# google/sentencepiece

Hardware: AMD Instinct MI355X
Metric: sentences/sec EncodeBatch, 32k unigram, MI355X (higher is better)
Workload: dtype u8 text -> i32 ids; f64 add / f32 store in the Viterbi relax

## Files before the change

sentencepiece_amd/csrc/api.cc:

```cpp
#include <hip/hip_runtime.h>

#include <cstdio>
#include <cstdlib>
#include <fcntl.h>
#include <sys/mman.h>
#include <sys/stat.h>
#include <sys/syscall.h>
#include <unistd.h>

#include <algorithm>
#include <cmath>
#include <condition_variable>
#include <cstring>
#include <fstream>
#include <functional>
#include <map>
#include <memory>
#include <mutex>
#include <thread>
#include <new>
#include <sstream>
#include <atomic>
#include <chrono>
#include <string>
// ... 281 lines not shown
  uint32_t dyn_list_cap = kDynListCapDefault;
  uint64_t nbest_budget = 32ull << 30;
  uint32_t nbest_hyps_min = 4096;
  uint32_t tile_min_lanes = 1;
  int32_t dx_npre = 0, dx_nsuf = 0, dx_pre[kMaxExtra] = {0}, dx_suf[kMaxExtra] = {0};
  bool dx_reverse = false;
  bool dx_unk = false;
  uint32_t compact_staged = 2048;
  bool no_direct = false;
  int fork_cus = 0;
  int fork_waves = 4;
  bool early_tail = false;
  bool no_overlap = false;
  bool no_ids16 = false;
  bool no_scan = false;
  bool no_word_dyn = false;
  bool memo_unsafe = false;
  bool force_word_dp = false;
  bool no_split = false;
  uint32_t split_min_raw = 576;
  bool split_own_launch = false;
  uint32_t split_tiles = 1;
  uint32_t split_per_byte = 4;
  uint32_t compact_big = kCompactBigIds;
  bool uw_exact = false;
  int uw_pipe = 1;
  bool no_uni_wave = false;
  uint32_t uni_wave_max = 0;
  int word_wgs = 1;
  uint64_t table_bytes = 0;
  uint64_t dn_table_bytes = 0;
  double load_ms = 0.0;
  int word_form = 3;
  int wordwave_waves = 14;
  int word_waves = 12;
  int tile_waves_override = 0;
  uint32_t lane_general_min_lanes = 0;
  uint32_t sub_buckets = kSubBuckets;
  int host_threads = 24;
  uint64_t host_chunk = 0;
  int reserve_cus = 0;
  uint32_t ring_override = 0;
  uint64_t stream_scratch_limit = 16ull << 30;
  bool wide_tcap = false;
  uint32_t main_max_raw = kStreamMainMaxRaw;
  LengthClass classes[kNumClasses];
};

namespace {

int Fail(spmx_handle *, int code, const std::string &msg) {
  t_error = msg;
  return code;
}
int FailHip(spmx_handle *h, hipError_t e, const char *what) {
  return Fail(h, kInternal, std::string(what) + ": " + hipGetErrorString(e));
}

#define HIP_OR_RETURN(h, expr)                                   \
  do {                                                           \
    hipError_t e_ = (expr);                                      \
    if (e_ != hipSuccess) return FailHip((h), e_, #expr);        \
  } while (0)

struct Lease {
  spmx_handle *h;
  std::unique_ptr<Workspace> ws;
// ... 385 lines not shown
  const bool fast_ok = StreamFastEligible(h->dev.flags) && !h->no_fast;
  const bool uds = (h->dev.flags & kNfHasUserDefined) != 0;
  uint32_t rcaps[kMaxClasses] = {0};
  for (int c = 0; c < ncls; ++c) rcaps[c] = cls[c].rcap;
  rcaps[ncls - 1] = cls[ncls - 1].rcap;
  const uint64_t max_raw = (0x7FFFFF00ull - 16) / h->dev.expand_max;
  auto record = [&](int slot, int which) -> hipError_t {
    return prof ? hipEventRecord(ws->ev[slot][which], stream) : hipSuccess;
  };
  auto scan_compact = [&]() -> int {
    ScanArgs sa{ws->d_counts.p, n32, ws->d_tile_sums.p, d_id_offsets};
    const uint32_t tiles = (n32 + kScanTile - 1) / kScanTile;
    HIP_OR_RETURN(h, LaunchScan(sa, static_cast<int>(tiles < static_cast<uint32_t>(wide) ? tiles : wide), stream));
    const uint32_t big = (n < 65536 || text_bytes > 160ull * n) ? h->compact_big : 0u;
    if (big) HIP_OR_RETURN(h, hipMemsetAsync(&ws->d_ctrl->big_count[0], 0, sizeof(uint32_t), stream));
    CompactArgs pa{ws->d_arena.p, ws->d_tmp_off.p, ws->d_counts.p, d_id_offsets, d_ids, d_ids ? ids_capacity : 0, n32, &ws->d_ctrl->status, h->compact_staged,
                   big, ws->d_big_list.p, &ws->d_ctrl->big_count[0]};
    const uint64_t cblocks = (n + 63) / 64;
    const uint64_t cgrid = cblocks < static_cast<uint64_t>(h->n_cu) * 32 ? cblocks : static_cast<uint64_t>(h->n_cu) * 32;
    HIP_OR_RETURN(h, LaunchCompact(pa, static_cast<int>(cgrid), stream));
    if (big) HIP_OR_RETURN(h, LaunchCompactBig(pa, h->n_cu * 4, stream));
    HIP_OR_RETURN(h, hipMemcpyAsync(ws->h_ctrl, ws->d_ctrl, offsetof(Ctrl, total_ids), hipMemcpyDeviceToHost, stream));
    HIP_OR_RETURN(h, hipMemcpyAsync(&ws->h_ctrl->total_ids, d_id_offsets + n, sizeof(uint64_t), hipMemcpyDeviceToHost, stream));
    HIP_OR_RETURN(h, hipStreamSynchronize(stream));
    return kOk;
  };
  uint64_t arena_cap_limit = 0;
  if (h->arena_first && arena_need > h->arena_first) { arena_need = h->arena_first; arena_cap_limit = h->arena_first; }
  const uint64_t arena_reserve = (h->arena_first || ws->reserve_text_bytes <= text_bytes) ? 0 :
      expand * ws->reserve_text_bytes + (10 + static_cast<uint64_t>(h->dev.n_prefix + h->dev.n_suffix)) * (ws->reserve_n > n ? ws->reserve_n : n) + 4096 +
      (direct ? (ws->reserve_text_bytes + (1 + static_cast<uint64_t>(h->dev.n_prefix + h->dev.n_suffix)) * (ws->reserve_n > n ? ws->reserve_n : n)) / (ids16 ? 2 : 1) + 8 : 0);
  for (int attempt = 0; attempt < 4; ++attempt) {
    uint64_t long_launches = 0;
    HIP_OR_RETURN(h, ws->d_arena.Reserve(arena_need > arena_reserve ? arena_need : arena_reserve));
    if (spans) HIP_OR_RETURN(h, ws->d_arena_tb.Reserve(ws->d_arena.cap));
    if (prof) HIP_OR_RETURN(h, hipEventRecord(ws->ev[kNumSlots][0], stream));
    HIP_OR_RETURN(h, hipMemsetAsync(ws->d_ctrl, 0, sizeof(Ctrl), stream));
    HIP_OR_RETURN(h, hipMemsetAsync(d_status, 0, n, stream));
    for (bool &u : ws->slot_used) u = false;
    uint32_t known[kMaxClasses] = {0};
    uint32_t gen_known[kMaxClasses] = {0};
    uint32_t align_known[kMaxClasses] = {0};
    uint64_t gen_total = 0;
    if (!direct) {
      if (int rc = RunClassify(h, ws, d_offsets, n32, stream, scanned ? d_text : nullptr, text_bytes, scanned ? gen_lists : nullptr); rc != kOk) return rc;
      HIP_OR_RETURN(h, hipMemcpyAsync(ws->h_ctrl->list_counts, ws->d_ctrl->list_counts,
                                      sizeof(ws->h_ctrl->list_counts) + sizeof(ws->h_ctrl->gen_counts),
                                      hipMemcpyDeviceToHost, stream));
      HIP_OR_RETURN(h, hipStreamSynchronize(stream));
      for (int c = 0; c < ncls; ++c) { known[c] = ws->h_ctrl->list_counts[c]; gen_known[c] = ws->h_ctrl->gen_counts[c]; gen_total += gen_known[c]; }
    } else {
      known[0] = n32;
    }
    EncodeArgs a{};
    a.dev = h->dev; a.text = d_text; a.offs = d_offsets;
    a.arena = ws->d_arena.p; a.arena_head = &ws->d_ctrl->arena_head;
    a.arena_cap = attempt == 0 && arena_cap_limit && arena_cap_limit < ws->d_arena.cap ? arena_cap_limit : ws->d_arena.cap;
    a.tmp_off = ws->d_tmp_off.p; a.counts = ws->d_counts.p; a.sent_status = d_status; a.status = &ws->d_ctrl->status;
    a.arena_tb = spans ? ws->d_arena_tb.p : nullptr;
    a.long_list = long_list; a.side = &ws->d_ctrl->side;
    a.lists = class_lists; a.over_list = over_list;
    a.n = n32;
    a.fast_ok = fast_ok ? 1u : 0u;
    a.no_lane_general = h->no_lane_general ? 1u : 0u;
    a.no_char_norm = h->char_norm_mode;
    int stream_waves_cap = 0;
// ... 227 lines not shown
        }
        int rc = kOk;
        for (int c = 0; c < ncls && rc == kOk; ++c)
          if (doc_known[c]) rc = long_launch(class_lists + static_cast<size_t>(c) * n, &ws->d_ctrl->list_counts[c], doc_known[c], true);
        if (rc == kOk) rc = general_pass(gen_lists, ws->d_ctrl->gen_counts, gen_known, false);
        if (forked) {
          if (rc != kOk) { (void)hipStreamSynchronize(ws->stream2); return rc; }
          if (hipError_t e = hipEventRecord(ws->ev_join, stream); e != hipSuccess) { (void)hipStreamSynchronize(ws->stream2); return FailHip(h, e, "hipEventRecord(join)"); }
          stream = main_stream;
          stream_waves_cap = 0;
          stream_cus_cap = 0;
        } else if (rc != kOk) {
          return rc;
        }
        a.lists = class_lists;
        d_list_counts = ws->d_ctrl->list_counts;
      }
    }
    auto fail_forked = [&](int rc) -> int {
      if (forked) (void)hipStreamSynchronize(ws->stream2);
      return rc;
    };
#define FORKED_OR_RETURN(expr) do { if (int rc_ = (expr); rc_ != kOk) return fail_forked(rc_); } while (0)
#define FORKED_HIP_OR_RETURN(expr) do { hipError_t e_ = (expr); if (e_ != hipSuccess) return fail_forked(FailHip(h, e_, #expr)); } while (0)
    if (word_ok) {
      const bool dyn = !h->no_word_dyn;
      word_pass = [&](int mode, int slot, int qi, uint32_t *out_lists, uint32_t *d_out_counts, uint32_t *out2_lists,
                           uint32_t *d_out2_counts) -> int {
        const bool dp = mode == 3;
        EncodeArgs wa = a;
        const bool wform = !dp && ((mode == 2 ? h->word_form & 2 : h->word_form & 1) != 0);
        int waves = dp ? 8 : wform ? h->wordwave_waves : h->word_waves;
        if (wform && mode == 2 && waves > static_cast<int>(kWwAgainMaxWaves)) waves = static_cast<int>(kWwAgainMaxWaves);
        while (wform && waves > 1 && WordWaveLdsBytes(static_cast<uint32_t>(waves)) > 160u * 1024u) --waves;
        uint64_t total = 0;
        for (int c = 0; c < ncls; ++c) total += known[c];
        if (total == 0) return kOk;
        uint64_t grid = static_cast<uint64_t>(h->n_cu - h->reserve_cus) * static_cast<uint64_t>(dp ? 1 : h->word_wgs);
        if (grid * waves * 64 > total) grid = (total + waves * 64 - 1) / (waves * 64);
        if (grid < 1) grid = 1;
        const uint64_t n_waves = grid * waves;
        wa.n_classes = static_cast<uint32_t>(ncls);
        uint32_t tile_base = 0;
        wa.direct = direct ? 1u : 0u;
        if (direct && mode != 2) wa.lists = nullptr;
        for (int c = ncls - 1; c >= 0; --c) {
          StreamClass &sc = wa.cls[c];
          sc = StreamClass{};
          sc.rcap = rcaps[c];
          if (direct) {
            sc.lane_shift = 6;
            sc.general = cls[c].rcap > kMaxStagedRaw ? 1u : 0u;
            if (c == 0) {
              sc.count = static_cast<uint32_t>(total);
              sc.tw = 64;
              sc.main_tiles = static_cast<uint32_t>((total + 63) / 64);
              sc.tile_base = 0;
              tile_base = sc.main_tiles;
            }
            continue;
          }
          if (known[c] == 0) continue;
          uint64_t tw = (static_cast<uint64_t>(known[c]) + n_waves - 1) / n_waves;
          if (tw > 64) tw = 64;
          if (tw < 1) tw = 1;
          sc.lane_shift = 6;
          sc.general = ((uni_class[c] && cls[c].rcap > kMaxStagedRaw) || cls[c].rcap > h->main_max_raw) ? 1u : 0u;
          sc.count = known[c];
          sc.tw = static_cast<uint32_t>(tw);
          sc.main_tiles = static_cast<uint32_t>((static_cast<uint64_t>(known[c]) + tw - 1) / tw);
          sc.tile_base = tile_base;
          tile_base += sc.main_tiles;
        }
        wa.total_main = tile_base;
        wa.q = &ws->d_ctrl->q[qi];
        wa.stats = &ws->d_ctrl->stats[kStatsPerClass * slot];
        wa.left_lists = out_lists;
        wa.left_counts = d_out_counts;
        wa.left2_lists = out2_lists;
        wa.left2_counts = d_out2_counts;
        wa.dyn_tag = ws->d_dyn_tag.p;
        wa.dyn_ent = ws->d_dyn_ent.p;
        wa.dyn_list = ws->d_dyn_list.p;
        wa.dyn_count = &ws->d_ctrl->dyn_count;
        wa.dyn_mask = h->dyn_slots - 1u;
        wa.dyn_cap = h->dyn_list_cap;
        wa.resume = ws->d_resume.p;
        wa.ids16 = ids16 ? 1u : 0u;
        wa.arena_first = (direct && mode != 2) ? direct_region : 0u;
        snprintf(ws->slot_name[slot], sizeof(ws->slot_name[slot]), "%s",
                 wform ? (wa.ids16 ? (mode == 2 ? "EncodeWordWaveAgainKernel<true>" : mode == 1 ? "EncodeWordWaveCollectKernel<true>" : "EncodeWordWaveKernel<true>")
                                   : (mode == 2 ? "EncodeWordWaveAgainKernel<false>" : mode == 1 ? "EncodeWordWaveCollectKernel<false>" : "EncodeWordWaveKernel<false>"))
                       : mode == 3 ? "EncodeWordDpKernel" : mode == 2 ? "EncodeWordAgainKernel" : mode == 1 ? "EncodeWordCollectKernel" : "EncodeWordKernel");
        HIP_OR_RETURN(h, record(slot, 0));
        if (wform) HIP_OR_RETURN(h, LaunchEncodeWordWave(mode, wa, static_cast<int>(grid), waves, WordWaveLdsBytes(waves), stream));
        else HIP_OR_RETURN(h, LaunchEncodeWord(mode, wa, static_cast<int>(grid), waves, WordLdsBytes(waves, dp), stream));
        HIP_OR_RETURN(h, record(slot, 1));
        ws->slot_used[slot] = true;
        return kOk;
      };
      auto read_counts = [&]() -> int {
        HIP_OR_RETURN(h, hipMemcpyAsync(ws->h_ctrl->left_counts, ws->d_ctrl->left_counts, sizeof(ws->h_ctrl->left_counts) + sizeof(uint32_t),
                                        hipMemcpyDeviceToHost, stream));
        HIP_OR_RETURN(h, hipStreamSynchronize(stream));
        return kOk;
      };
      uint64_t eligible = 0;
      for (int c = 0; c < ncls; ++c) if (cls[c].rcap <= h->main_max_raw) eligible += known[c];
      int left_at = 0;
      if (dyn) {
        FORKED_HIP_OR_RETURN(ws->d_dyn_tag.Reserve(h->dyn_slots));
        FORKED_HIP_OR_RETURN(ws->d_dyn_ent.Reserve(static_cast<size_t>(h->dyn_slots) * 4));
        FORKED_HIP_OR_RETURN(ws->d_dyn_list.Reserve(h->dyn_list_cap));
        FORKED_HIP_OR_RETURN(ws->d_resume.Reserve(n));
        FORKED_HIP_OR_RETURN(hipMemsetAsync(ws->d_dyn_tag.p, 0, static_cast<size_t>(h->dyn_slots) * sizeof(unsigned long long), stream));
        FORKED_OR_RETURN(word_pass(1, kSlotWord, 3, left_lists[0], ws->d_ctrl->left_counts[0], left_lists[1], ws->d_ctrl->left_counts[1]));
        FORKED_OR_RETURN(read_counts());
        for (int c = 0; c < ncls; ++c) { again_counts[c] = ws->h_ctrl->left_counts[0][c]; again_total += again_counts[c]; }
        again_words = ws->h_ctrl->dyn_count < h->dyn_list_cap ? ws->h_ctrl->dyn_count : h->dyn_list_cap;
        left_at = 1;
        if (again_total > 0) {
          uint32_t gone1[kMaxClasses] = {0};
          uint64_t gone1_total = 0;
          for (int c = 0; c < ncls; ++c) { gone1[c] = ws->h_ctrl->left_counts[1][c]; gone1_total += gone1[c]; }
          const bool early_tail = h->early_tail && direct && !forked && !h->no_overlap && gone1_total > 0;
          if (early_tail) {
            HIP_OR_RETURN(h, hipEventRecord(ws->ev_fork, stream));
            HIP_OR_RETURN(h, hipStreamWaitEvent(ws->stream2, ws->ev_fork, 0));
// ... 74 lines not shown
      }
    }
    if (ws->h_ctrl->side.long_count) {
      if (int rc = long_launch(long_list, &ws->d_ctrl->side.long_count, ws->h_ctrl->side.long_count); rc != kOk) return rc;
      extra = true;
    }
    if (extra) {
      if (int rc = scan_compact(); rc != kOk) return rc;
      if (ws->h_ctrl->status & kStArenaOverflow) {
        arena_need = ws->h_ctrl->arena_head + ws->h_ctrl->arena_head / 8 + 64;
        continue;
      }
    }
    if (prof) {
      HIP_OR_RETURN(h, hipEventRecord(ws->ev[kNumSlots][1], stream));
      HIP_OR_RETURN(h, hipStreamSynchronize(stream));
      Profile &p = ws->prof;
      p = Profile();
      p.n = kNumSlots;
      for (int c = 0; c < kNumSlots; ++c) {
        if (!ws->slot_used[c]) continue;
        memcpy(p.name[c], ws->slot_name[c], sizeof(p.name[c]));
        HIP_OR_RETURN(h, hipEventElapsedTime(&p.kernel_ms[c], ws->ev[c][0], ws->ev[c][1]));
        const unsigned long long *s = &ws->h_ctrl->stats[kStatsPerClass * c];
        p.sentences[c] = s[0];
        p.raw_bytes[c] = s[1];
        p.ids[c] = s[2];
        for (int k = 0; k < 5; ++k) p.cycles[c][k] = s[3 + k];
      }
      p.path[0] = ws->h_ctrl->side.n_backlog; p.path[1] = ws->h_ctrl->side.over_count; p.path[2] = ws->h_ctrl->side.long_count;
      p.path[3] = ws->h_ctrl->side.n_failed;
      p.path[4] = static_cast<uint64_t>(attempt);
      p.path[5] = long_launches;
      HIP_OR_RETURN(h, hipEventElapsedTime(&p.total_ms, ws->ev[kNumSlots][0], ws->ev[kNumSlots][1]));
      std::lock_guard<std::mutex> l(h->mu);
      h->prof = p;
    }
    if (total_ids) *total_ids = ws->h_ctrl->total_ids;
    if (n_failed) *n_failed = ws->h_ctrl->side.n_failed;
    if (ws->h_ctrl->total_ids > ids_capacity || !d_ids) {
      if (ws->h_ctrl->total_ids == 0) return kOk;
      return Fail(h, kResourceExhausted, "ids_capacity is too small");
    }
    if (spans && ws->h_ctrl->total_ids > 0) {
      const uint64_t total = ws->h_ctrl->total_ids;
      HIP_OR_RETURN(h, ws->d_tok_begin.Reserve(total));
      CompactArgs pa{ws->d_arena_tb.p, ws->d_tmp_off.p, ws->d_counts.p, d_id_offsets, ws->d_tok_begin.p, total, n32, nullptr, h->compact_staged,
                     h->compact_big, ws->d_big_list.p, &ws->d_ctrl->big_count[1]};
      if (h->compact_big) HIP_OR_RETURN(h, hipMemsetAsync(&ws->d_ctrl->big_count[1], 0, sizeof(uint32_t), stream));
      const uint64_t cblocks = (n + 63) / 64;
      const uint64_t cgrid = cblocks < static_cast<uint64_t>(h->n_cu) * 32 ? cblocks : static_cast<uint64_t>(h->n_cu) * 32;
      HIP_OR_RETURN(h, LaunchCompact(pa, static_cast<int>(cgrid), stream));
      if (h->compact_big) HIP_OR_RETURN(h, LaunchCompactBig(pa, h->n_cu * 4, stream));
      HIP_OR_RETURN(h, hipMemsetAsync(&ws->d_ctrl->status, 0, sizeof(uint32_t), stream));
      HIP_OR_RETURN(h, hipMemsetAsync(ws->d_ctrl->align_counts, 0, sizeof(ws->d_ctrl->align_counts), stream));
      HIP_OR_RETURN(h, hipMemsetAsync(&ws->d_ctrl->side.long_count, 0, sizeof(uint32_t), stream));
      AlignArgs base{};
      base.dev = h->dev; base.text = d_text; base.offs = d_offsets;
      base.id_offs = d_id_offsets; base.tok_begin = ws->d_tok_begin.p; base.begin = d_begin; base.end = d_end;
      base.nbegin = d_nbegin; base.nend = d_nbegin ? d_nend : nullptr;
      base.status = &ws->d_ctrl->status; base.list_cap = n32;
      bool prev = false;
      int c_staged = 0;
      while (c_staged < ncls && cls[c_staged].rcap <= kMaxStagedRaw) ++c_staged;
      for (int c = 0; c < c_staged; ++c) {
        const uint32_t cnt = known[c];
// ... 409 lines not shown
    if (const char *e = getenv("SPMX_TILE_MIN_LANES")) h->tile_min_lanes = static_cast<uint32_t>(atoi(e));
    if (const char *e = getenv("SPMX_NO_UNI_WAVE")) h->no_uni_wave = e[0] == '1';
    if (const char *e = getenv("SPMX_WORD_WGS")) { const int v = atoi(e); if (v >= 1 && v <= 4) h->word_wgs = v; }
    if (const char *e = getenv("SPMX_NO_BP_SHORT")) h->no_bp_short = e[0] == '1';
    if (const char *e = getenv("SPMX_WIDE_TCAP")) h->wide_tcap = e[0] == '1';
    if (const char *e = getenv("SPMX_SUB_BUCKETS")) {
      const int v = atoi(e);
      h->sub_buckets = static_cast<uint32_t>(v < 1 ? 1 : (v > kMaxSubBuckets ? kMaxSubBuckets : v));
    }
    if (const char *e = getenv("SPMX_LANE_GENERAL_MIN_LANES")) h->lane_general_min_lanes = static_cast<uint32_t>(atoi(e));
    if (const char *e = getenv("SPMX_STREAM_SCRATCH_MB")) h->stream_scratch_limit = static_cast<uint64_t>(atoll(e)) << 20;
    if (const char *e = getenv("SPMX_MAIN_MAX_RAW")) h->main_max_raw = static_cast<uint32_t>(atoll(e));
    if (const char *e = getenv("SPMX_FORCE_RING")) { const int v = atoi(e); if (v >= 16 && v <= 122) h->ring_override = static_cast<uint32_t>(v); }
#else
    {
      static const char *const kSeamOnly[] = {"SPMX_NO_WORD_DP", "SPMX_NBEST_HYPS_MIN", "SPMX_TILE_MIN_LANES",
          "SPMX_NO_UNI_WAVE", "SPMX_WORD_WGS", "SPMX_NO_BP_SHORT", "SPMX_WIDE_TCAP", "SPMX_SUB_BUCKETS", "SPMX_LANE_GENERAL_MIN_LANES",
          "SPMX_STREAM_SCRATCH_MB", "SPMX_MAIN_MAX_RAW", "SPMX_FORCE_RING", "SPMX_MEMO16_ONE"};
      static std::atomic<bool> warned{false};
      for (const char *v : kSeamOnly)
        if (getenv(v) && !warned.exchange(true))
          fprintf(stderr, "libspmx: %s is read by test-seam builds only (-DSPMX_TEST_SEAMS); this library ignores it\n", v);
    }
#endif
    if (const char *e = getenv("SPMX_NO_SPLIT")) h->no_split = e[0] == '1';
    if (const char *e = getenv("SPMX_SPLIT_MIN")) h->split_min_raw = static_cast<uint32_t>(atoll(e));
    if (const char *e = getenv("SPMX_SPLIT_LAUNCH")) h->split_own_launch = e[0] == '1';
    if (const char *e = getenv("SPMX_SPLIT_TILES")) { const int v = atoi(e); if (v >= 1 && v <= 16) h->split_tiles = static_cast<uint32_t>(v); }
    if (const char *e = getenv("SPMX_SPLIT_CANDS")) { const int v = atoi(e); if (v >= 1 && v <= 16) h->split_per_byte = static_cast<uint32_t>(v); }
    if (const char *e = getenv("SPMX_UW_PIPE")) h->uw_pipe = atoi(e);
    if (const char *e = getenv("SPMX_UNI_WAVE_MAX")) h->uni_wave_max = static_cast<uint32_t>(atoll(e));
    if (const char *e = getenv("SPMX_WORD_WAVE")) { const int v = atoi(e); if (v >= 0 && v <= 3) h->word_form = v; }
    if (const char *e = getenv("SPMX_WORDWAVE_WAVES")) { const int v = atoi(e); if (v >= 1 && v <= 16) h->wordwave_waves = v; }
    if (const char *e = getenv("SPMX_WORD_WAVES")) { const int v = atoi(e); if (v >= 1 && v <= 16) h->word_waves = v; }
    if (const char *e = getenv("SPMX_ARENA_FIRST")) h->arena_first = static_cast<uint64_t>(atoll(e));
    if (const char *e = getenv("SPMX_NO_LANE_GENERAL")) h->no_lane_general = e[0] == '1';
    if (const char *e = getenv("SPMX_NO_CHAR_NORM")) h->char_norm_mode = e[0] == '1' ? 1u : 0u;
    if (const char *e = getenv("SPMX_CHAR_NORM_ALWAYS")) { if (e[0] == '1') h->char_norm_mode = 2u; }
    if (const char *e = getenv("SPMX_TILE_WAVES")) h->tile_waves_override = atoi(e);
    if (const char *e = getenv("SPMX_RESERVE_CUS")) { const int v = atoi(e); if (v >= 0 && v < h->n_cu) h->reserve_cus = v; }
    if (const char *e = getenv("SPMX_HOST_THREADS")) { const int v = atoi(e); h->host_threads = v < 1 ? 1 : (v > 64 ? 64 : v); }
    if (const char *e = getenv("SPMX_HOST_CHUNK")) { const long long v = atoll(e); if (v >= 1024) h->host_chunk = static_cast<uint64_t>(v); }
    if (const char *e = getenv("SPMX_CLASSES")) {
      int c = 0;
      const char *p = e;
      while (*p && c < kNumClasses) {
        char *q = nullptr;
        const unsigned long r = strtoul(p, &q, 10);
        if (q == p || *q != ':') break;
        p = q + 1;
        const unsigned long nn = strtoul(p, &q, 10);
        if (q == p) break;
        h->classes[c++] = LengthClass{static_cast<uint32_t>(r), static_cast<uint32_t>(nn)};
        p = *q == ',' ? q + 1 : q;
      }
    }
    t_upload_bytes = 0;
    if (int rc = UploadTables(nullptr, h.get(), h->tables, &h->dev); rc != kOk) return rc;
    const uint64_t model_table_bytes = t_upload_bytes;
    if (int rc = UploadDenormTables(h.get()); rc != kOk) return rc;
    h->table_bytes = t_upload_bytes;
    h->dn_table_bytes = t_upload_bytes - model_table_bytes;
    h->load_ms = std::chrono::duration<double, std::milli>(std::chrono::steady_clock::now() - t_load0).count();
    if (!h->model.self_test.empty())
      if (int rc = RunSelfTest(h.get()); rc != kOk) return rc;
    *out = h.release();
// ... 2551 lines not shown
}

int spmx_handle_info(const spmx_handle *h, uint64_t *table_bytes, double *load_ms) {
  if (!h) return kInvalidArgument;
  if (table_bytes) *table_bytes = h->table_bytes;
  if (load_ms) *load_ms = h->load_ms;
  return kOk;
}

int spmx_last_phase_cycles(const spmx_handle *h, uint64_t *cycles) {
  if (!h) return 0;
  for (int c = 0; c < h->prof.n; ++c)
    for (int k = 0; k < 5; ++k) cycles[5 * c + k] = h->prof.cycles[c][k];
  return h->prof.n;
}

int spmx_last_profile_name(const spmx_handle *h, int slot, char *out, uint64_t cap) {
  if (!h || slot < 0 || slot >= h->prof.n || !out || !cap) return 0;
  snprintf(out, cap, "%s", h->prof.name[slot]);
  return static_cast<int>(strlen(h->prof.name[slot]));
}

int spmx_last_profile(const spmx_handle *h, float *kernel_ms, uint64_t *sentences, uint64_t *raw_bytes, uint64_t *ids,
                      uint64_t *bytes, uint64_t *path, float *total_ms) {
  if (!h) return 0;
  const Profile &p = h->prof;
  for (int c = 0; c < p.n; ++c) {
    if (kernel_ms) kernel_ms[c] = p.kernel_ms[c];
    if (sentences) sentences[c] = p.sentences[c];
    if (raw_bytes) raw_bytes[c] = p.raw_bytes[c];
    if (ids) ids[c] = p.ids[c];
    if (bytes) bytes[c] = p.raw_bytes[c] + 16 * p.sentences[c] + 4 * p.ids[c];
  }
  if (path) for (int k = 0; k < 6; ++k) path[k] = p.path[k];
  if (total_ms) *total_ms = p.total_ms;
  return p.n;
}

}

#ifdef SPMX_WAVE_API
#include "../../tests/emu/emu_launch_charword.h"
#include "../../tests/emu/emu_launch_idtext.h"
#include "../../tests/emu/emu_launch_tokentext.h"
#include "../../tests/emu/emu_launch_piececount.h"
#include "../../tests/emu/emu_launch_latticecsr.h"
#endif
```

sentencepiece_amd/csrc/kernels.h:

```cpp
#ifndef SPMX_KERNELS_H_
#define SPMX_KERNELS_H_

#ifndef SPMX_WAVE_API
#include "wave.h"
#endif
#include <math.h>

#include "dev.h"

namespace spmx {

enum : uint32_t {
  kStArenaOverflow = 1u << 0,
  kStTooLong = 1u << 1,
  kStInternal = 1u << 2,
};
enum : uint32_t { kSsOk = 0, kSsResourceExhausted = 8, kSsOutOfRange = 11, kSsInternal = 13 };

constexpr int kMaxClasses = 8;

struct StreamClass {
  uint32_t rcap;
  uint32_t tcap;
  uint32_t lane_shift;
// ... 36 lines not shown
  uint32_t *long_list;
  SideLists *side;
  const uint32_t *lists;
  uint32_t *over_list;
  StreamQueue *q;
  uint8_t *slab;
  uint64_t slab_bytes;
  uint32_t n;
  uint32_t n_classes;
  uint32_t total_main;
  uint32_t bp_short;
  uint32_t ring;
  uint32_t fast_ok;
  uint32_t no_lane_general;
  uint32_t private_bytes;
  uint32_t split_ring;
  uint32_t match_rows;
  uint32_t no_char_norm;
  StreamClass cls[kMaxClasses];
  uint32_t *left_lists;
  uint32_t *left_counts;
  uint32_t *left2_lists;
  uint32_t *left2_counts;
  unsigned long long *dyn_tag;
  U4 *dyn_ent;
  uint32_t *dyn_list;
  uint32_t *dyn_count;
  uint32_t dyn_mask;
  uint32_t dyn_cap;
  U4 *resume;
  uint32_t ids16;
  uint32_t direct;
  uint64_t arena_first;
  const uint32_t *list;
  const uint32_t *list_count;
  uint32_t *next_list;
  uint32_t *next_count;
  uint32_t rcap, ncap;
};

constexpr int kStatsPerClass = 8;
constexpr uint32_t kTokEnd = 0x8000u;

SPMX_DEVICE uint32_t DartsOffset(uint32_t u) { return (u >> 10) << ((u & (1u << 9)) >> 6); }

SPMX_DEVICE int OneCharLenDev(uint32_t c) {
  const uint32_t h = c >> 4;
  return h < 12 ? 1 : (h < 14 ? 2 : (h == 14 ? 3 : 4));
}
SPMX_DEVICE uint32_t SpByteOf(const SpmxDev &d) { return (d.flags & kNfCompressSp) ? kSpByte : 0x100u; }

SPMX_DEVICE int wave_excl_scan(int v, int lane, int *total) {
  int incl = v;
#pragma unroll
  for (int d = 1; d < 64; d <<= 1) {
    const int up = wv::shfl_up(incl, d);
    if (lane >= d) incl += up;
  }
  *total = wv::shfl(incl, 63);
  return incl - v;
}

SPMX_DEVICE uint64_t resolve_chain(int base, int step, bool valid, int *next_start) {
  const uint64_t m1 = wv::ballot(valid && step == 1);
  const uint64_t m2 = wv::ballot(valid && step == 2);
  const uint64_t m3 = wv::ballot(valid && step == 3);
// ... 1094 lines not shown
```

sentencepiece_amd/csrc/kernels_wordwave.h:

```cpp
#ifndef SPMX_KERNELS_WORDWAVE_H_
#define SPMX_KERNELS_WORDWAVE_H_

namespace spmx {

constexpr uint32_t kWwRing = 4096u;
constexpr uint32_t kWwRingPad = 32u;
constexpr uint32_t kWwUnits = kWwRing / 16u;
constexpr uint32_t kWwMaskBytes = (kWwUnits + 4u) * 2u + 8u;
constexpr uint32_t kWwRecs = 128u + 512u;
constexpr uint32_t kWwMaxLen = 65536u;
constexpr uint32_t kWwPerWave = kWwRing + kWwRingPad + kWwMaskBytes + kWwRecs * 4u + 64u * 16u + 64u * 8u + 5u * 64u * 4u;
static_assert(kWwPerWave % 16u == 0u, "per-wave LDS blocks keep 16-byte alignment");
constexpr uint32_t kWwAgainMaxWaves = 12u;
constexpr uint32_t kWwAgain = 1u, kWwGone = 2u;
constexpr uint32_t kWwKeyMaskBytes = 640u;
constexpr uint32_t kWwShared = kWwKeyMaskBytes + kWordHotSlots * 16u + kUallBuckets * 2u;
SPMX_HD constexpr bool kWwHotIn(int mode) { return mode == 2; }
SPMX_HD inline uint32_t WordWaveLdsBytes(uint32_t waves) { return kWwShared + waves * kWwPerWave; }

struct __attribute__((packed, aligned(2))) U64H { uint32_t lo, hi; };

SPMX_DEVICE uint32_t space_mask16(const Q4 &v) {
  auto m4 = [](uint32_t z) -> uint32_t { return (((z >> 7) & 0x01010101u) * 0x10204080u) >> 28; };
  return m4(space_flags(v.x)) | (m4(space_flags(v.y)) << 4) | (m4(space_flags(v.z)) << 8) | (m4(space_flags(v.w)) << 12);
}
SPMX_DEVICE uint32_t key_dword_n(uint32_t text, int n) {
  const uint32_t m = n >= 4 ? 0xFFFFFFFFu : (n <= 0 ? 0u : (1u << (8 * n)) - 1u);
  return key_dword(text, m);
}

struct DynWalked { uint32_t hit, n, bound, lim; U4 ia, ib; };
SPMX_DEVICE DynWalked dyn_walk(const unsigned long long *dyn_tag, const U4 *dyn_ent, uint32_t dyn_mask, uint32_t k0,
                                    uint32_t k1, uint32_t k2, uint32_t k3, unsigned long long tag) {
  DynWalked w{0u, 0u, 0u, 0u, U4{0, 0, 0, 0}, U4{0, 0, 0, 0}};
  uint32_t sl = static_cast<uint32_t>(tag >> 32) & dyn_mask;
#pragma unroll 1
  for (uint32_t t = 1; t < kDynProbes; ++t) {
    sl = (sl + 1u) & dyn_mask;
    const unsigned long long g = dyn_tag[sl];
    if (g == 0ull) break;
    if (g != tag) continue;
    const U4 d0 = dyn_ent[4u * sl], d1 = dyn_ent[4u * sl + 1u];
    if (d0.x == k0 && d0.y == k1 && d0.z == k2 && d0.w == k3 && d1.x == 1u) {
      w.hit = 1u; w.n = d1.y; w.bound = d1.z; w.lim = d1.w;
      w.ia = dyn_ent[4u * sl + 2u];
      w.ib = dyn_ent[4u * sl + 3u];
      wv::opaque(w.ia.x); wv::opaque(w.ia.y); wv::opaque(w.ia.z); wv::opaque(w.ia.w);
      wv::opaque(w.ib.x); wv::opaque(w.ib.y); wv::opaque(w.ib.z); wv::opaque(w.ib.w);
    }
    break;
  }
  return w;
}

struct WwStage {
  uint32_t cnt;
  uint32_t P, j;
  uint32_t L;
  uint32_t k0, k1, k2, k3;
  uint32_t hz, hw;
  uint32_t e0x, e0y, e0z, e0w, e1x, e1y, e1z, e1w;
  uint32_t tg_lo, tg_hi;
  uint32_t warm;
  uint32_t d0x, d0y, d0z, d0w, d1x, d1y, d1z, d1w, d2x, d2y, d2z, d2w;
};
constexpr uint32_t kWwHit16 = 0x100u;

template <int MODE, bool H16>
SPMX_DEVICE void encode_wordwave_block(const EncodeArgs &a, unsigned char *smem) {
  const int lane = wv::lane();
  const SpmxDev &d = a.dev;
  Q4 *masks = reinterpret_cast<Q4 *>(smem);
  U4 *hot = reinterpret_cast<U4 *>(smem + kWwKeyMaskBytes);
  uint16_t *disp = reinterpret_cast<uint16_t *>(smem + kWwKeyMaskBytes + kWordHotSlots * 16u);
  unsigned char *mine_lds = smem + kWwShared + static_cast<uint32_t>(wv::wave_in_block()) * kWwPerWave;
  uint8_t *ring = mine_lds;
  uint16_t *smask = reinterpret_cast<uint16_t *>(mine_lds + kWwRing + kWwRingPad);
  uint32_t *recq = reinterpret_cast<uint32_t *>(mine_lds + kWwRing + kWwRingPad + kWwMaskBytes);
  U4 *sent = reinterpret_cast<U4 *>(recq + kWwRecs);
  U2 *sent_ua = reinterpret_cast<U2 *>(sent + 64);
  uint32_t *s_nids = reinterpret_cast<uint32_t *>(sent_ua + 64), *s_stat = s_nids + 64, *s_first = s_stat + 64;
  uint32_t *s_n0 = s_first + 64, *s_x0 = s_n0 + 64;
  {
    if (lane < 18) {
      const uint32_t L = static_cast<uint32_t>(lane);
      auto m = [&](uint32_t i) -> uint32_t { return L >= 4u * i + 4u ? 0xFFFFFFFFu : (L <= 4u * i ? 0u : (1u << (8u * (L - 4u * i))) - 1u); };
      masks[2 * lane] = Q4{m(0), m(1), m(2), m(3)};
      masks[2 * lane + 1] = Q4{kWordKeyPad & ~m(0), kWordKeyPad & ~m(1), kWordKeyPad & ~m(2), kWordKeyPad & ~m(3)};
    }
    if (kWwHotIn(MODE)) for (uint32_t k = static_cast<uint32_t>(lane); k < kWordHotSlots; k += 64u) hot[k] = d.uhot2[k];
    for (uint32_t k = static_cast<uint32_t>(lane); k < kUallBuckets; k += 64u) disp[k] = d.udisp[k];
    wv::sync();
  }
  const U4 *__restrict__ uall = d.uall;
  const uint32_t mall = d.uall_mask;
  const bool perfect = d.uall_perfect != 0u;
  const int n_extra = d.n_prefix + d.n_suffix;
  const bool keep_ws = (d.flags & kNfRemoveExtraWs) == 0;
  const bool any_word = (d.flags & kNfWordLocalNorm) != 0;
  const uint64_t tbase = reinterpret_cast<uint64_t>(a.text);
  WaveCounters tc;
  if (MODE != kWmDyn && a.arena_first != 0u && wv::block_id() == 0 && wv::wave_in_block() == 0 && lane == 0)
    wv::atomic_add(a.arena_head, static_cast<unsigned long long>(a.arena_first));
  WwStage SA{}, SB{};
  uint32_t dyn_warm = 0u;
  for (;;) {
    const unsigned long long cs = wv::clock();
    uint32_t c = 0, first = 0, ucnt = 0, got = 0;
    if (lane == 0) got = next_tile(a, &c, &first, &ucnt) ? 1u : 0u;
    got = wv::shfl(got, 0);
    if (!got) break;
    c = wv::shfl(c, 0); first = wv::shfl(first, 0); ucnt = wv::shfl(ucnt, 0);
    const bool direct = a.direct != 0u;
    const uint32_t *list = a.lists ? a.lists + static_cast<uint64_t>(c) * a.n : nullptr;
    const bool have = static_cast<uint32_t>(lane) < ucnt;
    uint32_t sid = 0;
    uint64_t beg = 0, l64 = 0;
    if (have) {
      sid = list ? list[first + static_cast<uint32_t>(lane)] : first + static_cast<uint32_t>(lane);
      beg = a.offs[sid];
      l64 = a.offs[sid + 1] - beg;
    }
    uint32_t cl = c;
    if (direct) {
      cl = a.n_classes - 1u;
      for (int k = static_cast<int>(a.n_classes) - 2; k >= 0; --k) if (l64 <= a.cls[k].rcap) cl = static_cast<uint32_t>(k);
    }
    const bool mine = have && !a.cls[cl].general && l64 <= kWwMaxLen;
    uint32_t p0 = 0u, n0 = 0u, x0 = 0u;
    uint64_t src0 = 0;
    if (MODE == kWmDyn && mine) {
      const uint64_t t = a.tmp_off[sid];
      src0 = ((t & kTmpOffHalf) ? (t & ~kTmpOffHalf) : (H16 ? 2ull * t : t)) + static_cast<uint64_t>(d.n_prefix);
      const U4 rs = a.resume[sid];
      const float bf0 = wv::bits_to_float(rs.z);
      if (rs.x < l64 && rs.y <= rs.x && bf0 >= 0.f && bf0 < 16777216.f) { p0 = rs.x; n0 = rs.y; x0 = static_cast<uint32_t>(bf0); }
    }
    const bool fixed = direct && list == nullptr && MODE != kWmDyn;
    const uint64_t room = !have ? 0ull : static_cast<uint64_t>(n_extra) + ((fixed || mine) ? l64 + 1ull : 0ull);
    uint64_t rtotal = 0;
    wave_excl_scan64(room, lane, &rtotal);
    uint64_t base = 0;
    bool overflow;
    if (fixed) {
      const uint64_t o0 = a.offs[0];
// ... 485 lines not shown
```

sentencepiece_amd/processor.py:

```python
import ctypes as C
import os

import numpy as np

from . import _capi

_PYEXT = [False, None]


def _pyext():
    if _PYEXT[0] is False:
        try:
            from . import _spmx_py
            _PYEXT[1] = _spmx_py
        except ImportError:
            _PYEXT[1] = None
        _PYEXT[0] = True
    return _PYEXT[1]

_OK = 0
_RESOURCE_EXHAUSTED = 8
_PROTO_TYPES = ("serialized_proto", "proto", "immutable_proto")


# ... 1537 lines not shown
        self._check(self._lib.spmx_write_vocabulary(self._h, counts.ctypes.data, os.fsencode(out_path), C.byref(nl)))
        return sentences, ids, int(nl.value)

    def SetProfiling(self, enabled):
        self._need()
        self._lib.spmx_set_profiling(self._h, 1 if enabled else 0)

    def HandleInfo(self):
        tb, ms = C.c_uint64(0), C.c_double(0.0)
        self._check(self._lib.spmx_handle_info(self._h, C.byref(tb), C.byref(ms)))
        return {"table_bytes": int(tb.value), "load_ms": float(ms.value)}

    def LastProfile(self):
        self._need()
        ms = np.zeros(8, dtype=np.float32)
        sent, raw, ids, byt = (np.zeros(8, dtype=np.uint64) for _ in range(4))
        path = np.zeros(8, dtype=np.uint64)
        tot = C.c_float(0)
        k = self._lib.spmx_last_profile(self._h, ms.ctypes.data, sent.ctypes.data, raw.ctypes.data, ids.ctypes.data,
                                        byt.ctypes.data, path.ctypes.data, C.byref(tot))
        cyc = np.zeros(80, dtype=np.uint64)
        self._lib.spmx_last_phase_cycles(self._h, cyc.ctypes.data)
        names = []
        for c in range(k):
            buf = C.create_string_buffer(64)
            self._lib.spmx_last_profile_name(self._h, c, buf, 64)
            names.append(buf.value.decode())
        return dict(classes=[dict(kernel=names[c], kernel_ms=float(ms[c]), sentences=int(sent[c]), raw_bytes=int(raw[c]),
                                  ids=int(ids[c]), bytes=int(byt[c]),
                                  phase_cycles=dict(zip(("load", "normalize", "segment", "emit", "search_trips"),
                                                        (int(x) for x in cyc[5 * c:5 * c + 5]))))
                             for c in range(k)],
                    path=dict(backlog=int(path[0]), overflow=int(path[1]), long=int(path[2]), failed=int(path[3]),
                              arena_retries=int(path[4]), long_launches=int(path[5])),
                    total_ms=float(tot.value))
```

Baseline: 2.454 billion.

## Statically assign most word-wave tiles and trim per-mode LDS to fit more waves

Lets most tiles in the word-wave kernel be handed out statically by wave index with a fixed stride. Only the remaining tail goes through the global atomic cursor, which cuts contention on that cursor. LDS sizing is now per mode: the hot-slot table and two per-wave scratch arrays are kept only where they are used, so the default wave count per block rises from 14 to 16. A static split can leave load imbalance on the front portion, and it adds profiling fields that report the chosen wave counts.

```diff
diff --git a/sentencepiece_amd/csrc/api.cc b/sentencepiece_amd/csrc/api.cc
--- a/sentencepiece_amd/csrc/api.cc
+++ b/sentencepiece_amd/csrc/api.cc
@@ -337,7 +337,8 @@
   uint64_t dn_table_bytes = 0;
   double load_ms = 0.0;
   int word_form = 3;
-  int wordwave_waves = 14;
+  int wordwave_waves = 16;
+  double static_tiles_frac = 0.875;
   int word_waves = 12;
   int tile_waves_override = 0;
   uint32_t lane_general_min_lanes = 0;
@@ -789,6 +790,7 @@
       (direct ? (ws->reserve_text_bytes + (1 + static_cast<uint64_t>(h->dev.n_prefix + h->dev.n_suffix)) * (ws->reserve_n > n ? ws->reserve_n : n)) / (ids16 ? 2 : 1) + 8 : 0);
   for (int attempt = 0; attempt < 4; ++attempt) {
     uint64_t long_launches = 0;
+    uint64_t word_waves[2] = {0, 0};
     HIP_OR_RETURN(h, ws->d_arena.Reserve(arena_need > arena_reserve ? arena_need : arena_reserve));
     if (spans) HIP_OR_RETURN(h, ws->d_arena_tb.Reserve(ws->d_arena.cap));
     if (prof) HIP_OR_RETURN(h, hipEventRecord(ws->ev[kNumSlots][0], stream));
@@ -1082,7 +1084,7 @@
         const bool wform = !dp && ((mode == 2 ? h->word_form & 2 : h->word_form & 1) != 0);
         int waves = dp ? 8 : wform ? h->wordwave_waves : h->word_waves;
         if (wform && mode == 2 && waves > static_cast<int>(kWwAgainMaxWaves)) waves = static_cast<int>(kWwAgainMaxWaves);
-        while (wform && waves > 1 && WordWaveLdsBytes(static_cast<uint32_t>(waves)) > 160u * 1024u) --waves;
+        while (wform && waves > 1 && WordWaveLdsBytes(mode, static_cast<uint32_t>(waves)) > 160u * 1024u) --waves;
         uint64_t total = 0;
         for (int c = 0; c < ncls; ++c) total += known[c];
         if (total == 0) return kOk;
@@ -1123,6 +1125,10 @@
           tile_base += sc.main_tiles;
         }
         wa.total_main = tile_base;
+        wa.static_tiles = 0;
+        wa.static_stride = static_cast<uint32_t>(n_waves);
+        if (wform && direct && mode != 2 && h->static_tiles_frac > 0.0)
+          wa.static_tiles = static_cast<uint32_t>(static_cast<uint64_t>(h->static_tiles_frac * static_cast<double>(tile_base)) / n_waves * n_waves);
         wa.q = &ws->d_ctrl->q[qi];
         wa.stats = &ws->d_ctrl->stats[kStatsPerClass * slot];
         wa.left_lists = out_lists;
@@ -1142,8 +1148,9 @@
                  wform ? (wa.ids16 ? (mode == 2 ? "EncodeWordWaveAgainKernel<true>" : mode == 1 ? "EncodeWordWaveCollectKernel<true>" : "EncodeWordWaveKernel<true>")
                                    : (mode == 2 ? "EncodeWordWaveAgainKernel<false>" : mode == 1 ? "EncodeWordWaveCollectKernel<false>" : "EncodeWordWaveKernel<false>"))
                        : mode == 3 ? "EncodeWordDpKernel" : mode == 2 ? "EncodeWordAgainKernel" : mode == 1 ? "EncodeWordCollectKernel" : "EncodeWordKernel");
+        if (wform) word_waves[mode == 2 ? 1 : 0] = static_cast<uint64_t>(waves);
         HIP_OR_RETURN(h, record(slot, 0));
-        if (wform) HIP_OR_RETURN(h, LaunchEncodeWordWave(mode, wa, static_cast<int>(grid), waves, WordWaveLdsBytes(waves), stream));
+        if (wform) HIP_OR_RETURN(h, LaunchEncodeWordWave(mode, wa, static_cast<int>(grid), waves, WordWaveLdsBytes(mode, static_cast<uint32_t>(waves)), stream));
         else HIP_OR_RETURN(h, LaunchEncodeWord(mode, wa, static_cast<int>(grid), waves, WordLdsBytes(waves, dp), stream));
         HIP_OR_RETURN(h, record(slot, 1));
         ws->slot_used[slot] = true;
@@ -1284,6 +1291,7 @@
       p.path[3] = ws->h_ctrl->side.n_failed;
       p.path[4] = static_cast<uint64_t>(attempt);
       p.path[5] = long_launches;
+      p.path[6] = word_waves[0]; p.path[7] = word_waves[1];
       HIP_OR_RETURN(h, hipEventElapsedTime(&p.total_ms, ws->ev[kNumSlots][0], ws->ev[kNumSlots][1]));
       std::lock_guard<std::mutex> l(h->mu);
       h->prof = p;
@@ -1759,6 +1767,7 @@
     if (const char *e = getenv("SPMX_UNI_WAVE_MAX")) h->uni_wave_max = static_cast<uint32_t>(atoll(e));
     if (const char *e = getenv("SPMX_WORD_WAVE")) { const int v = atoi(e); if (v >= 0 && v <= 3) h->word_form = v; }
     if (const char *e = getenv("SPMX_WORDWAVE_WAVES")) { const int v = atoi(e); if (v >= 1 && v <= 16) h->wordwave_waves = v; }
+    if (const char *e = getenv("SPMX_STATIC_TILES")) { const double v = atof(e); if (v >= 0.0 && v <= 1.0) h->static_tiles_frac = v; }
     if (const char *e = getenv("SPMX_WORD_WAVES")) { const int v = atoi(e); if (v >= 1 && v <= 16) h->word_waves = v; }
     if (const char *e = getenv("SPMX_ARENA_FIRST")) h->arena_first = static_cast<uint64_t>(atoll(e));
     if (const char *e = getenv("SPMX_NO_LANE_GENERAL")) h->no_lane_general = e[0] == '1';
@@ -4376,7 +4385,7 @@
     if (ids) ids[c] = p.ids[c];
     if (bytes) bytes[c] = p.raw_bytes[c] + 16 * p.sentences[c] + 4 * p.ids[c];
   }
-  if (path) for (int k = 0; k < 6; ++k) path[k] = p.path[k];
+  if (path) for (int k = 0; k < 8; ++k) path[k] = p.path[k];
   if (total_ms) *total_ms = p.total_ms;
   return p.n;
 }
diff --git a/sentencepiece_amd/csrc/kernels.h b/sentencepiece_amd/csrc/kernels.h
--- a/sentencepiece_amd/csrc/kernels.h
+++ b/sentencepiece_amd/csrc/kernels.h
@@ -92,6 +92,7 @@
   uint32_t ids16;
   uint32_t direct;
   uint64_t arena_first;
+  uint32_t static_tiles, static_stride;
   const uint32_t *list;
   const uint32_t *list_count;
   uint32_t *next_list;
diff --git a/sentencepiece_amd/csrc/kernels_wordwave.h b/sentencepiece_amd/csrc/kernels_wordwave.h
--- a/sentencepiece_amd/csrc/kernels_wordwave.h
+++ b/sentencepiece_amd/csrc/kernels_wordwave.h
@@ -9,14 +9,18 @@
 constexpr uint32_t kWwMaskBytes = (kWwUnits + 4u) * 2u + 8u;
 constexpr uint32_t kWwRecs = 128u + 512u;
 constexpr uint32_t kWwMaxLen = 65536u;
-constexpr uint32_t kWwPerWave = kWwRing + kWwRingPad + kWwMaskBytes + kWwRecs * 4u + 64u * 16u + 64u * 8u + 5u * 64u * 4u;
-static_assert(kWwPerWave % 16u == 0u, "per-wave LDS blocks keep 16-byte alignment");
+SPMX_HD constexpr uint32_t kWwPerWave(int mode) {
+  return kWwRing + kWwRingPad + kWwMaskBytes + kWwRecs * 4u + 64u * 16u + 64u * 8u + 3u * 64u * 4u + (mode == 2 ? 2u * 64u * 4u : 0u);
+}
+static_assert(kWwPerWave(0) % 16u == 0u && kWwPerWave(1) % 16u == 0u && kWwPerWave(2) % 16u == 0u,
+              "per-wave LDS blocks keep 16-byte alignment");
 constexpr uint32_t kWwAgainMaxWaves = 12u;
 constexpr uint32_t kWwAgain = 1u, kWwGone = 2u;
 constexpr uint32_t kWwKeyMaskBytes = 640u;
-constexpr uint32_t kWwShared = kWwKeyMaskBytes + kWordHotSlots * 16u + kUallBuckets * 2u;
 SPMX_HD constexpr bool kWwHotIn(int mode) { return mode == 2; }
-SPMX_HD inline uint32_t WordWaveLdsBytes(uint32_t waves) { return kWwShared + waves * kWwPerWave; }
+SPMX_HD constexpr uint32_t kWwShared(int mode) { return kWwKeyMaskBytes + (kWwHotIn(mode) ? kWordHotSlots * 16u : 0u) + kUallBuckets * 2u; }
+static_assert(kWwShared(0) % 16u == 0u && kWwShared(2) % 16u == 0u, "the shared tables keep 16-byte alignment");
+SPMX_HD inline uint32_t WordWaveLdsBytes(int mode, uint32_t waves) { return kWwShared(mode) + waves * kWwPerWave(mode); }
 
 struct __attribute__((packed, aligned(2))) U64H { uint32_t lo, hi; };
 
@@ -66,21 +70,36 @@
 };
 constexpr uint32_t kWwHit16 = 0x100u;
 
+template <int MODE>
+SPMX_DEVICE U4 ww_next_tile(const EncodeArgs &a, int lane, uint32_t own_tile) {
+  uint32_t t = own_tile;
+  if (MODE == kWmDyn || own_tile >= a.static_tiles) {
+    uint32_t v = 0;
+    if (lane == 0) v = wv::atomic_add(&a.q->main_cursor, 1u);
+    t = wv::uniform((MODE != kWmDyn ? a.static_tiles : 0u) + wv::shfl(v, 0));
+  }
+  if (t >= a.total_main) return U4{0u, 0u, 0u, 0u};
+  int k = static_cast<int>(a.n_classes) - 1;
+  while (k > 0 && !(t >= a.cls[k].tile_base && t - a.cls[k].tile_base < a.cls[k].main_tiles)) --k;
+  const uint32_t first = (t - a.cls[k].tile_base) * a.cls[k].tw, left = a.cls[k].count - first;
+  return U4{1u, static_cast<uint32_t>(k), first, left < a.cls[k].tw ? left : a.cls[k].tw};
+}
+
 template <int MODE, bool H16>
 SPMX_DEVICE void encode_wordwave_block(const EncodeArgs &a, unsigned char *smem) {
   const int lane = wv::lane();
   const SpmxDev &d = a.dev;
   Q4 *masks = reinterpret_cast<Q4 *>(smem);
   U4 *hot = reinterpret_cast<U4 *>(smem + kWwKeyMaskBytes);
-  uint16_t *disp = reinterpret_cast<uint16_t *>(smem + kWwKeyMaskBytes + kWordHotSlots * 16u);
-  unsigned char *mine_lds = smem + kWwShared + static_cast<uint32_t>(wv::wave_in_block()) * kWwPerWave;
+  uint16_t *disp = reinterpret_cast<uint16_t *>(smem + kWwShared(MODE) - kUallBuckets * 2u);
+  unsigned char *mine_lds = smem + kWwShared(MODE) + static_cast<uint32_t>(wv::wave_in_block()) * kWwPerWave(MODE);
   uint8_t *ring = mine_lds;
   uint16_t *smask = reinterpret_cast<uint16_t *>(mine_lds + kWwRing + kWwRingPad);
   uint32_t *recq = reinterpret_cast<uint32_t *>(mine_lds + kWwRing + kWwRingPad + kWwMaskBytes);
   U4 *sent = reinterpret_cast<U4 *>(recq + kWwRecs);
   U2 *sent_ua = reinterpret_cast<U2 *>(sent + 64);
   uint32_t *s_nids = reinterpret_cast<uint32_t *>(sent_ua + 64), *s_stat = s_nids + 64, *s_first = s_stat + 64;
-  uint32_t *s_n0 = s_first + 64, *s_x0 = s_n0 + 64;
+  uint32_t *s_n0 = MODE == kWmDyn ? s_first + 64 : nullptr, *s_x0 = MODE == kWmDyn ? s_first + 128 : nullptr;
   {
     if (lane < 18) {
       const uint32_t L = static_cast<uint32_t>(lane);
@@ -104,13 +123,13 @@
     wv::atomic_add(a.arena_head, static_cast<unsigned long long>(a.arena_first));
   WwStage SA{}, SB{};
   uint32_t dyn_warm = 0u;
+  uint32_t own_tile = wv::uniform(static_cast<uint32_t>(wv::block_id() * wv::waves_per_block() + wv::wave_in_block()));
   for (;;) {
     const unsigned long long cs = wv::clock();
-    uint32_t c = 0, first = 0, ucnt = 0, got = 0;
-    if (lane == 0) got = next_tile(a, &c, &first, &ucnt) ? 1u : 0u;
-    got = wv::shfl(got, 0);
-    if (!got) break;
-    c = wv::shfl(c, 0); first = wv::shfl(first, 0); ucnt = wv::shfl(ucnt, 0);
+    const U4 tl = ww_next_tile<MODE>(a, lane, own_tile);
+    if (!tl.x) break;
+    if (MODE != kWmDyn && own_tile < a.static_tiles) own_tile += a.static_stride;
+    const uint32_t c = tl.y, first = tl.z, ucnt = tl.w;
     const bool direct = a.direct != 0u;
     const uint32_t *list = a.lists ? a.lists + static_cast<uint64_t>(c) * a.n : nullptr;
     const bool have = static_cast<uint32_t>(lane) < ucnt;
diff --git a/sentencepiece_amd/processor.py b/sentencepiece_amd/processor.py
--- a/sentencepiece_amd/processor.py
+++ b/sentencepiece_amd/processor.py
@@ -1593,5 +1593,6 @@
                                                         (int(x) for x in cyc[5 * c:5 * c + 5]))))
                              for c in range(k)],
                     path=dict(backlog=int(path[0]), overflow=int(path[1]), long=int(path[2]), failed=int(path[3]),
-                              arena_retries=int(path[4]), long_launches=int(path[5])),
+                              arena_retries=int(path[4]), long_launches=int(path[5]),
+                              word_waves_first=int(path[6]), word_waves_second=int(path[7])),
                     total_ms=float(tot.value))
```

New measurement: 2.649 billion, median of 6. 7.9% higher.
